# lorenzrichter/path-space-PDE-solver

Measured on AMD Instinct MI355X. Metric: trajectory-timesteps/sec (K*N/s), d=100 HJB log-variance training iteration, higher is better.
Workload: dtype f32 (f16x3 split products: every matrix product as three f16 MFMAs, fp32 accumulate; state / sums fp32)

## Files before the change

path-space-pde-solver_amd/csrc/hjb_kernels.h:

```cpp
#pragma once
#include <cstdlib>
#include <type_traits>
#include <hip/hip_runtime.h>
#include <stdint.h>

namespace psp {

typedef float f32x4 __attribute__((ext_vector_type(4)));

struct HjbArgs {
    const float* params;
    const float* x0;
    const float* y0;
    const float* xi;
    float* path;
    float* D;
    float* XN;
    double* fwd_partial;
    const float* drift;
    const float* sigma;
    const float* runcost;
    const float* term;
    const double* sums;
    float* grad_partial;
// ... 190 lines not shown
    constexpr int NCH = cdiv(KS, CH);
    lane = opaque_i(lane);
    float buf[2][CH * MB];
#pragma unroll
    for (int kk = 0; kk < CH; ++kk)
#pragma unroll
        for (int mb = 0; mb < MB; ++mb)
            if (kk < KS) buf[0][kk * MB + mb] = wlds[(mb * KS + kk) * 64 + lane];
#pragma unroll
    for (int c = 0; c < NCH; ++c) {
        if (c + 1 < NCH) {
#pragma unroll
            for (int kk = 0; kk < CH; ++kk)
#pragma unroll
                for (int mb = 0; mb < MB; ++mb) {
                    const int ks = (c + 1) * CH + kk;
                    if (ks < KS) buf[(c + 1) & 1][kk * MB + mb] = wlds[(mb * KS + ks) * 64 + lane];
                }
        }
#pragma unroll
        for (int kk = 0; kk < CH; ++kk) {
            const int ks = c * CH + kk;
            if (ks < KS) {
                const float bop = in[ks >> 2][ks & 3];
#pragma unroll
                for (int mb = 0; mb < MB; ++mb) acc[mb] = mfma16(buf[c & 1][kk * MB + mb], bop, acc[mb]);
            }
        }
        __builtin_amdgcn_sched_barrier(kFenceMask);
    }
}

typedef __bf16 bf16x8 __attribute__((ext_vector_type(8)));
template <class F>
__device__ __forceinline__ void stage_aop_bf16(float* dstf, int MB, int NS, int tid, int nthr, F src) {
    bf16x8* dst = reinterpret_cast<bf16x8*>(dstf);
    const int total = MB * NS * 64;
    for (int idx = tid; idx < total; idx += nthr) {
        const int lane = idx & 63, t = idx >> 6;
        const int S = t % NS, mb = t / NS;
        const int i = lane & 15, g = lane >> 4;
        const int row = 16 * mb + 4 * (i & 3) + (i >> 2);
        bf16x8 v;
#pragma unroll
        for (int e = 0; e < 8; ++e) v[e] = (__bf16)src(row, 32 * S + (e < 4 ? 4 * e : 16 + 4 * (e - 4)) + g);
        dst[idx] = v;
    }
}
template <int MB, int INB>
__device__ __forceinline__ void gemm_Tb(f32x4 (&acc)[MB], const float* wlds, const f32x4 (&in)[INB], int lane) {
    constexpr int NS = (INB + 1) / 2;
    const bf16x8* tbl = reinterpret_cast<const bf16x8*>(wlds) + opaque_i(lane);
#pragma unroll
    for (int S = 0; S < NS; ++S) {
        bf16x8 b;
#pragma unroll
        for (int e = 0; e < 4; ++e) {
            b[e] = (__bf16)in[2 * S][e];
            b[4 + e] = (2 * S + 1 < INB) ? (__bf16)in[(2 * S + 1 < INB) ? 2 * S + 1 : 0][e] : (__bf16)0.0f;
        }
#pragma unroll
        for (int mb = 0; mb < MB; ++mb)
            acc[mb] = __builtin_amdgcn_mfma_f32_16x16x32_bf16(tbl[(mb * NS + S) * 64], b, acc[mb], 0, 0, 0);
    }
}

typedef _Float16 f16x8 __attribute__((ext_vector_type(8)));
typedef _Float16 f16x4 __attribute__((ext_vector_type(4)));
constexpr float kSplitScale = 2048.0f, kSplitInv = 1.0f / 2048.0f;
template <int KS, int INB>
struct SplitGeo {
    static constexpr int NS = INB / 2;
    static constexpr bool ODD = (INB & 1) != 0;
    static constexpr int NKR = ODD ? KS - 8 * NS : 0;
    static constexpr bool ODD_F32 = ODD && NKR <= 1;
    static constexpr bool ODD_H16 = ODD && NKR > 1;
    static constexpr int per_mb = NS * 512 + (ODD_F32 ? 64 : 0) + (ODD_H16 ? 256 : 0);
    static constexpr int floats(int MB) { return MB * per_mb; }
};
__device__ __forceinline__ void split_f16(float v, _Float16& hi, _Float16& lo) {
    hi = (_Float16)v;
    lo = (_Float16)((v - (float)hi) * kSplitScale);
}

typedef _Float16 f16x2 __attribute__((ext_vector_type(2)));
typedef float f32x2 __attribute__((ext_vector_type(2)));
__device__ __forceinline__ void split_pair(float a, float b, f16x2& hi, f16x2& lo) {
    const f32x2 v = {a, b};
    hi = __builtin_convertvector(v, f16x2);
    const f32x2 s = v * kSplitScale;
    lo[0] = (_Float16)__builtin_fmaf((float)hi[0], -kSplitScale, s[0]);
    lo[1] = (_Float16)__builtin_fmaf((float)hi[1], -kSplitScale, s[1]);
}
__device__ __forceinline__ void split4c(const f32x4& u, f16x4& hi, f16x4& lo) {
#pragma unroll
    for (int e = 0; e < 4; ++e) {
        _Float16 h, l;
        split_f16(u[e], h, l);
        hi[e] = h; lo[e] = l;
    }
}
__device__ __forceinline__ void split4(const f32x4& u, f16x4& hi, f16x4& lo) {
#if defined(PSP_SPLIT_CLASSIC) && PSP_SPLIT_CLASSIC
#pragma unroll
    for (int e = 0; e < 4; ++e) {
        _Float16 h, l;
        split_f16(u[e], h, l);
        hi[e] = h; lo[e] = l;
    }
    return;
#endif
    f16x2 h, l;
    split_pair(u[0], u[1], h, l); hi[0] = h[0]; hi[1] = h[1]; lo[0] = l[0]; lo[1] = l[1];
    split_pair(u[2], u[3], h, l); hi[2] = h[0]; hi[3] = h[1]; lo[2] = l[0]; lo[3] = l[1];
}
__device__ __forceinline__ void split8(const f32x4& u0, const f32x4& u1, f16x8& hi, f16x8& lo) {
#if defined(PSP_SPLIT_CLASSIC) && PSP_SPLIT_CLASSIC
#pragma unroll
    for (int e = 0; e < 4; ++e) {
        _Float16 h, l;
        split_f16(u0[e], h, l);
        hi[e] = h; lo[e] = l;
        split_f16(u1[e], h, l);
        hi[4 + e] = h; lo[4 + e] = l;
    }
    return;
#endif
    f16x2 h, l;
    split_pair(u0[0], u0[1], h, l); hi[0] = h[0]; hi[1] = h[1]; lo[0] = l[0]; lo[1] = l[1];
    split_pair(u0[2], u0[3], h, l); hi[2] = h[0]; hi[3] = h[1]; lo[2] = l[0]; lo[3] = l[1];
    split_pair(u1[0], u1[1], h, l); hi[4] = h[0]; hi[5] = h[1]; lo[4] = l[0]; lo[5] = l[1];
    split_pair(u1[2], u1[3], h, l); hi[6] = h[0]; hi[7] = h[1]; lo[6] = l[0]; lo[7] = l[1];
}
__device__ __forceinline__ void split_pair_u(float a, float b, f16x2& hi, f16x2& lo) {
    const f32x2 v = {a, b};
    hi = __builtin_convertvector(v, f16x2);
    lo[0] = (_Float16)__builtin_fmaf((float)hi[0], -1.0f, v[0]);
    lo[1] = (_Float16)__builtin_fmaf((float)hi[1], -1.0f, v[1]);
}
__device__ __forceinline__ void split8u(const f32x4& u0, const f32x4& u1, f16x8& hi, f16x8& lo) {
#if defined(PSP_SPLIT_CLASSIC) && PSP_SPLIT_CLASSIC
#pragma unroll
    for (int e = 0; e < 4; ++e) {
        _Float16 h = (_Float16)u0[e];
        hi[e] = h; lo[e] = (_Float16)(u0[e] - (float)h);
        h = (_Float16)u1[e];
        hi[4 + e] = h; lo[4 + e] = (_Float16)(u1[e] - (float)h);
    }
    return;
#endif
    f16x2 h, l;
    split_pair_u(u0[0], u0[1], h, l); hi[0] = h[0]; hi[1] = h[1]; lo[0] = l[0]; lo[1] = l[1];
    split_pair_u(u0[2], u0[3], h, l); hi[2] = h[0]; hi[3] = h[1]; lo[2] = l[0]; lo[3] = l[1];
    split_pair_u(u1[0], u1[1], h, l); hi[4] = h[0]; hi[5] = h[1]; lo[4] = l[0]; lo[5] = l[1];
    split_pair_u(u1[2], u1[3], h, l); hi[6] = h[0]; hi[7] = h[1]; lo[6] = l[0]; lo[7] = l[1];
}
template <int KS, int INB, class F>
__device__ __forceinline__ void stage_aop_x3(float* dstf, int MB, int tid, int nthr, F src) {
    using SG = SplitGeo<KS, INB>;
    if constexpr (SG::NS > 0) {
        for (int idx = tid; idx < MB * SG::NS * 64; idx += nthr) {
            const int lane = idx & 63, t = idx >> 6;
            const int S = t % SG::NS, mb = t / SG::NS;
            const int i = lane & 15, g = lane >> 4;
            const int row = 16 * mb + 4 * (i & 3) + (i >> 2);
            f16x8 hi, lo;
#pragma unroll
            for (int e = 0; e < 8; ++e) {
                _Float16 h, l;
                split_f16(src(row, 32 * S + (e < 4 ? 4 * e : 16 + 4 * (e - 4)) + g), h, l);
                hi[e] = h; lo[e] = l;
            }
            f16x8* p = reinterpret_cast<f16x8*>(dstf + mb * SG::per_mb + S * 512);
            p[lane] = hi; p[64 + lane] = lo;
        }
    }
    if constexpr (SG::ODD) {
        for (int idx = tid; idx < MB * 64; idx += nthr) {
            const int lane = idx & 63, mb = idx >> 6;
            const int i = lane & 15, g = lane >> 4;
            const int row = 16 * mb + 4 * (i & 3) + (i >> 2);
            if constexpr (SG::ODD_F32) {
                dstf[mb * SG::per_mb + SG::NS * 512 + lane] = src(row, 32 * SG::NS + g);
            } else {
                f16x4 hi, lo;
#pragma unroll
                for (int e = 0; e < 4; ++e) {
                    _Float16 h, l;
                    split_f16(src(row, 32 * SG::NS + 4 * e + g), h, l);
                    hi[e] = h; lo[e] = l;
                }
                f16x4* p = reinterpret_cast<f16x4*>(dstf + mb * SG::per_mb + SG::NS * 512);
                p[lane] = hi; p[64 + lane] = lo;
            }
        }
    }
}
struct NoBetween { __device__ __forceinline__ void operator()(int) const {} };
template <int MB, int KS, int INB, int CU = 2, class BT = NoBetween>
__device__ __forceinline__ void gemm_Tx(f32x4 (&acc)[MB], const float* wlds, const f32x4 (&in)[INB], int lane, BT between = BT()) {
    constexpr int kFence = std::is_same<BT, NoBetween>::value ? kFenceMask : 0;
    using SG = SplitGeo<KS, INB>;
    constexpr int NS = SG::NS;
    static_assert(MB * SG::per_mb * 4 <= 65536, "table exceeds the 16-bit ds_read immediate offset");
    lane = opaque_i(lane);
    f32x4 corr[MB];
#pragma unroll
    for (int mb = 0; mb < MB; ++mb) corr[mb] = f32x4{0.f, 0.f, 0.f, 0.f};
    if constexpr (NS > 0) {
        const f16x8* tbl = reinterpret_cast<const f16x8*>(wlds) + lane;
        constexpr int NU = NS * MB, R = 2 * CU, PF = R - 1;
        f16x8 ah[R], al[R];
#pragma unroll
        for (int u = 0; u < PF; ++u)
            if (u < NU) {
                ah[u % R] = tbl[((u % MB) * SG::per_mb + (u / MB) * 512) / 4];
                al[u % R] = tbl[((u % MB) * SG::per_mb + (u / MB) * 512) / 4 + 64];
            }
        f16x8 bh, bl;
#pragma unroll
        for (int u = 0; u < NU; ++u) {
            if (u + PF < NU) {
                const int v = u + PF;
                ah[v % R] = tbl[((v % MB) * SG::per_mb + (v / MB) * 512) / 4];
                al[v % R] = tbl[((v % MB) * SG::per_mb + (v / MB) * 512) / 4 + 64];
            }
            const int S = u / MB, mb = u % MB;
            if (mb == 0) split8(in[2 * S], in[2 * S + 1], bh, bl);
            acc[mb] = __builtin_amdgcn_mfma_f32_16x16x32_f16(ah[u % R], bh, acc[mb], 0, 0, 0);
            corr[mb] = __builtin_amdgcn_mfma_f32_16x16x32_f16(ah[u % R], bl, corr[mb], 0, 0, 0);
            corr[mb] = __builtin_amdgcn_mfma_f32_16x16x32_f16(al[u % R], bh, corr[mb], 0, 0, 0);
            between(u);
            __builtin_amdgcn_sched_barrier(kFence);
        }
    }
    if constexpr (SG::ODD_F32) {
        const float bop = in[INB - 1][0];
#pragma unroll
        for (int mb = 0; mb < MB; ++mb) acc[mb] = mfma16(wlds[mb * SG::per_mb + NS * 512 + lane], bop, acc[mb]);
    }
    if constexpr (SG::ODD_H16) {
        f16x4 bh, bl;
        split4c(in[INB - 1], bh, bl);
#pragma unroll
        for (int mb = 0; mb < MB; ++mb) {
            const f16x4* p = reinterpret_cast<const f16x4*>(wlds + mb * SG::per_mb + NS * 512) + lane;
            const f16x4 a_hi = p[0], a_lo = p[64];
            acc[mb] = __builtin_amdgcn_mfma_f32_16x16x16f16(a_hi, bh, acc[mb], 0, 0, 0);
            corr[mb] = __builtin_amdgcn_mfma_f32_16x16x16f16(a_hi, bl, corr[mb], 0, 0, 0);
            corr[mb] = __builtin_amdgcn_mfma_f32_16x16x16f16(a_lo, bh, corr[mb], 0, 0, 0);
        }
    }
#pragma unroll
    for (int mb = 0; mb < MB; ++mb) acc[mb] = acc[mb] + kSplitInv * corr[mb];
}

template <int INB>
__device__ __forceinline__ void split_panel8(const f32x4 (&in)[INB], f16x8 (&bh)[INB / 2 > 0 ? INB / 2 : 1], f16x8 (&bl)[INB / 2 > 0 ? INB / 2 : 1]) {
#pragma unroll
    for (int S = 0; S < INB / 2; ++S) split8(in[2 * S], in[2 * S + 1], bh[S], bl[S]);
}
template <int MB, int KS, int INB, int CU = 2, class BT = NoBetween>
__device__ __forceinline__ void gemm_Txs(f32x4 (&acc)[MB], const float* wlds, const f16x8 (&bh)[INB / 2 > 0 ? INB / 2 : 1],
                                         const f16x8 (&bl)[INB / 2 > 0 ? INB / 2 : 1], const f32x4& last, int lane, BT between = BT()) {
    constexpr int kFence = std::is_same<BT, NoBetween>::value ? kFenceMask : 0;
    using SG = SplitGeo<KS, INB>;
    constexpr int NS = SG::NS;
    lane = opaque_i(lane);
    f32x4 corr[MB];
#pragma unroll
    for (int mb = 0; mb < MB; ++mb) corr[mb] = f32x4{0.f, 0.f, 0.f, 0.f};
    if constexpr (NS > 0) {
        const f16x8* tbl = reinterpret_cast<const f16x8*>(wlds) + lane;
        constexpr int NU = NS * MB, R = 2 * CU, PF = R - 1;
        f16x8 ah[R], al[R];
#pragma unroll
        for (int u = 0; u < PF; ++u)
            if (u < NU) {
                ah[u % R] = tbl[((u % MB) * SG::per_mb + (u / MB) * 512) / 4];
                al[u % R] = tbl[((u % MB) * SG::per_mb + (u / MB) * 512) / 4 + 64];
            }
#pragma unroll
        for (int u = 0; u < NU; ++u) {
            if (u + PF < NU) {
                const int v = u + PF;
                ah[v % R] = tbl[((v % MB) * SG::per_mb + (v / MB) * 512) / 4];
                al[v % R] = tbl[((v % MB) * SG::per_mb + (v / MB) * 512) / 4 + 64];
            }
            const int S = u / MB, mb = u % MB;
            acc[mb] = __builtin_amdgcn_mfma_f32_16x16x32_f16(ah[u % R], bh[S], acc[mb], 0, 0, 0);
            corr[mb] = __builtin_amdgcn_mfma_f32_16x16x32_f16(ah[u % R], bl[S], corr[mb], 0, 0, 0);
            corr[mb] = __builtin_amdgcn_mfma_f32_16x16x32_f16(al[u % R], bh[S], corr[mb], 0, 0, 0);
            between(u);
            __builtin_amdgcn_sched_barrier(kFence);
        }
    }
    if constexpr (SG::ODD_F32) {
        const float bop = last[0];
#pragma unroll
        for (int mb = 0; mb < MB; ++mb) acc[mb] = mfma16(wlds[mb * SG::per_mb + NS * 512 + lane], bop, acc[mb]);
    }
    if constexpr (SG::ODD_H16) {
        f16x4 b4h, b4l;
        split4c(last, b4h, b4l);
#pragma unroll
        for (int mb = 0; mb < MB; ++mb) {
            const f16x4* p = reinterpret_cast<const f16x4*>(wlds + mb * SG::per_mb + NS * 512) + lane;
            const f16x4 a_hi = p[0], a_lo = p[64];
            acc[mb] = __builtin_amdgcn_mfma_f32_16x16x16f16(a_hi, b4h, acc[mb], 0, 0, 0);
            corr[mb] = __builtin_amdgcn_mfma_f32_16x16x16f16(a_hi, b4l, corr[mb], 0, 0, 0);
            corr[mb] = __builtin_amdgcn_mfma_f32_16x16x16f16(a_lo, b4h, corr[mb], 0, 0, 0);
        }
    }
#pragma unroll
    for (int mb = 0; mb < MB; ++mb) acc[mb] = acc[mb] + kSplitInv * corr[mb];
}

__device__ __forceinline__ float qsum(float v) {
    v += __shfl_xor(v, 16);
    v += __shfl_xor(v, 32);
    return v;
}
__device__ __forceinline__ float jsumf(float v) {
    v += __shfl_xor(v, 1);
    v += __shfl_xor(v, 2);
    v += __shfl_xor(v, 4);
    v += __shfl_xor(v, 8);
    return v;
}
__device__ __forceinline__ double jsum(double v) {
    v += __shfl_xor(v, 1);
    v += __shfl_xor(v, 2);
    v += __shfl_xor(v, 4);
    v += __shfl_xor(v, 8);
    return v;
}

__device__ __forceinline__ float tanh_f32(float x) {
    const float e = __builtin_amdgcn_exp2f(fabsf(x) * 2.8853900817779268f);
    const float big = fmaf(-2.0f, __builtin_amdgcn_rcpf(e + 1.0f), 1.0f);
    return copysignf(big, x);
}
__device__ __forceinline__ f32x4 tanh4(f32x4 v) {
    f32x4 o;
    o[0] = tanh_f32(v[0]); o[1] = tanh_f32(v[1]); o[2] = tanh_f32(v[2]); o[3] = tanh_f32(v[3]);
    return o;
}

__device__ __forceinline__ f32x4 relu4n(f32x4 v) {
    f32x4 o;
    o[0] = v[0] < 0.f ? 0.f : v[0]; o[1] = v[1] < 0.f ? 0.f : v[1]; o[2] = v[2] < 0.f ? 0.f : v[2]; o[3] = v[3] < 0.f ? 0.f : v[3];
    return o;
}

template <int D, int H>
struct Geo {
    static constexpr int DB = cdiv(D, 16), HB = cdiv(H, 16);
    static constexpr int KSD = cdiv(D, 4), KSH = cdiv(H, 4);
    static constexpr int oW1 = 0, ob1 = H * (D + 1), oW2 = ob1 + H, ob2 = oW2 + H * H, oW3 = ob2 + H,
                         ob3 = oW3 + D * H, P = ob3 + D;
    static constexpr int tbl(int MB, int KS, int INB) { return MB * (KS > 4 * ((INB + 1) / 2) ? KS : 4 * ((INB + 1) / 2)) * 64; }
    static constexpr int fW1 = 0, fW2 = fW1 + tbl(HB, KSD, DB), fW3 = fW2 + tbl(HB, KSH, HB),
                         fVec = fW3 + tbl(DB, KSH, HB);
    static_assert(D <= 12 || H <= 12 || fVec == (HB * KSD + HB * KSH + DB * KSH) * 64, "only inputs of <= 12 features change the carve");
    static constexpr int vb1 = fVec, vw1t = vb1 + HB * 16, vb2 = vw1t + HB * 16, vb3 = vb2 + HB * 16,
                         vdr = vb3 + DB * 16, vrun = vdr + DB * 16, vterm = vrun + DB * 16,
                         fRed = vterm + DB * 16;
    static constexpr int fA = fRed + 64;
    static constexpr int fB_dense_off = DB * KSD * 64;
    static constexpr int xW1 = 0, xW2 = xW1 + SplitGeo<KSD, DB>::floats(HB), xW3 = xW2 + SplitGeo<KSH, HB>::floats(HB),
                         xVec = xW3 + SplitGeo<KSH, HB>::floats(DB), xA = xVec + (fA - fVec);
    static constexpr int xB_dense_off = SplitGeo<KSD, DB>::floats(DB);
    static int fwd_x3_lds_floats(int drift_kind, int sigma_kind) {
        return xA + (drift_kind == DRIFT_DENSE ? xB_dense_off : 0) + (sigma_kind == SIGMA_DENSE ? xB_dense_off : 0);
    }
    static int fwd_lds_floats(int drift_kind, int sigma_kind) {
        return fA + (drift_kind == DRIFT_DENSE ? fB_dense_off : 0) + (sigma_kind == SIGMA_DENSE ? fB_dense_off : 0);
    }
    static constexpr int pX = 0, pH1 = 4 * DB * 64, pH2 = pH1 + 4 * HB * 64, pXi = pH2 + 4 * HB * 64, PB = pXi + 4 * DB * 64;
    static constexpr int WH = (HB >= 4) ? 4 : (HB >= 2 ? 2 : 1);
    static constexpr int WD = 4 / WH;
    static constexpr int NIB = cdiv(HB, WH);
    static constexpr int NOBD = cdiv(DB, WD);
    static constexpr int NOBH = cdiv(HB, WD);
    static constexpr int EXB = KSD * 64 + 4 * HB * 64;
    static int bwd2_lds_floats() { return HB * KSD * 64 + 2 * 4 * EXB; }
};

template <int D, int H, int MODE = 0, int FAST_ = 0>
__global__ __launch_bounds__(512) void hjb_fwd_kernel(const HjbArgs a) {
    PSP_COND_EXIT(a);
    constexpr bool FAST = FAST_ != 0, SPEC = FAST_ >= 2;
    const int k_drift = SPEC ? (int)DRIFT_DENSE : a.drift_kind;
    const int k_sigma = FAST_ == 3 ? (int)SIGMA_IDENT : SPEC ? (int)SIGMA_DENSE : a.sigma_kind;
    const int k_run = SPEC ? (int)RUN_ZERO : a.runcost_kind, k_loss = SPEC ? (int)LOSS_LOGVAR : a.loss_kind;
    const int k_store = a.store_path;
    const bool k_adaptive = SPEC ? true : (a.adaptive != 0);
    const uint32_t iter_now = a.iter_dev ? *a.iter_dev : a.iter;
    using G = Geo<D, H>;
    constexpr int DB = G::DB, HB = G::HB, KSD = G::KSD, KSH = G::KSH;
    constexpr bool BF16 = MODE == 1, X3 = MODE == 2;
    constexpr int oW1 = X3 ? G::xW1 : G::fW1, oW2 = X3 ? G::xW2 : G::fW2, oW3 = X3 ? G::xW3 : G::fW3;
    constexpr int VEC = X3 ? G::xVec : G::fVec;
    constexpr int VSH = VEC - G::fVec;
    extern __shared__ __attribute__((aligned(16))) float lds[];
    const int tid = threadIdx.x, nthr = blockDim.x;
    const int lane = tid & 63, wave = tid >> 6, nwave = nthr >> 6;
    const int j = lane & 15, q = lane >> 4;

    const float* __restrict__ P = a.params;
    auto stage_net = [&](float* dst, int MB, int KS, int INB, auto src) {
        if constexpr (BF16) stage_aop_bf16(dst, MB, (INB + 1) / 2, tid, nthr, src);
        else stage_aop(dst, MB, KS, tid, nthr, src);
    };
    auto w1src = [&](int row, int col) { return (row < H && col < D) ? P[G::oW1 + row * (D + 1) + 1 + col] : 0.f; };
    auto w2src = [&](int row, int col) { return (row < H && col < H) ? P[G::oW2 + row * H + col] : 0.f; };
    auto w3src = [&](int row, int col) { return (row < D && col < H) ? P[G::oW3 + row * H + col] : 0.f; };
    if constexpr (X3) {
        stage_aop_x3<KSD, DB>(lds + oW1, HB, tid, nthr, w1src);
        stage_aop_x3<KSH, HB>(lds + oW2, HB, tid, nthr, w2src);
        stage_aop_x3<KSH, HB>(lds + oW3, DB, tid, nthr, w3src);
    } else {
        stage_net(lds + oW1, HB, KSD, DB, w1src);
        stage_net(lds + oW2, HB, KSH, HB, w2src);
        stage_net(lds + oW3, DB, KSH, HB, w3src);
    }
    float* ldsA = lds + G::fA + VSH;
    float* ldsB = ldsA + (k_drift == DRIFT_DENSE ? (X3 ? G::xB_dense_off : G::fB_dense_off) : 0);
    if (k_drift == DRIFT_DENSE) {
        const float dt = a.dt;
        const float* __restrict__ A = a.drift;
        auto asrc = [&](int row, int col) { return (row < D && col < D) ? dt * A[row * D + col] : 0.f; };
        if constexpr (X3) stage_aop_x3<KSD, DB>(ldsA, DB, tid, nthr, asrc);
        else stage_aop(ldsA, DB, KSD, tid, nthr, asrc);
    }
    if (k_sigma == SIGMA_DENSE) {
        const float* __restrict__ B = a.sigma;
        auto bsrc = [&](int row, int col) { return (row < D && col < D) ? B[row * D + col] : 0.f; };
        if constexpr (X3) stage_aop_x3<KSD, DB>(ldsB, DB, tid, nthr, bsrc);
        else stage_aop(ldsB, DB, KSD, tid, nthr, bsrc);
    }
    stage_vec(lds + VSH + G::vb1, HB, tid, nthr, [&](int f) { return f < H ? P[G::ob1 + f] : 0.f; });
    stage_vec(lds + VSH + G::vw1t, HB, tid, nthr, [&](int f) { return f < H ? P[G::oW1 + f * (D + 1)] : 0.f; });
    stage_vec(lds + VSH + G::vb2, HB, tid, nthr, [&](int f) { return f < H ? P[G::ob2 + f] : 0.f; });
    stage_vec(lds + VSH + G::vb3, DB, tid, nthr, [&](int f) { return f < D ? P[G::ob3 + f] : 0.f; });
    stage_vec(lds + VSH + G::vdr, DB, tid, nthr, [&](int f) {
        return (f < D && (k_drift == DRIFT_DIAG || k_drift == DRIFT_DWELL)) ? a.drift[f] : 0.f; });
    stage_vec(lds + VSH + G::vrun, DB, tid, nthr, [&](int f) {
        return (f < D && k_run == RUN_DIAGQ) ? a.runcost[f] : 0.f; });
    stage_vec(lds + VSH + G::vterm, DB, tid, nthr, [&](int f) { return f < D ? a.term[f] : 0.f; });
    __syncthreads();

    const int t16 = blockIdx.x * nwave + wave;
    const bool wave_valid = t16 < a.ntile16;
    const int k = t16 * 16 + j;
    const bool kvalid = wave_valid && k < a.K_local;
    const uint32_t kglob = (uint32_t)(a.k_offset + k);
    const float dt = a.dt, sqdt = a.sqdt;

    const float store_cxi = SPEC ? 1.f : ((k_store == 3) ? 0.f : 1.f);
    const float store_cz = SPEC ? 0.f : ((k_store == 3) ? 1.f : (k_store == 2 ? -a.sqdt : (k_adaptive ? 0.f : a.sqdt)));
    const bool do_store = FAST ? true : (k_store != 0);
    double sD = 0.0, sD2 = 0.0;
    if (wave_valid) {
        const f32x4* vecs0 = reinterpret_cast<const f32x4*>(lds + VEC) + q;
        const f32x4* vterm = vecs0 + (G::vterm - G::fVec) / 4;

        f32x4 X[DB];
#pragma unroll
        for (int b = 0; b < DB; ++b) {
#pragma unroll
            for (int r = 0; r < 4; ++r) {
                const int f = 16 * b + 4 * r + q;
                const float v = a.x0[(size_t)(kvalid ? k : 0) * a.x0_stride + (f < D ? f : D - 1)];
                X[b][r] = (f < D && kvalid) ? v : 0.f;
            }
        }
        float Y = a.y0 ? a.y0[0] : 0.f;
        float Fsum = 0.f, ULsum = 0.f;
#ifdef PSP_STAMPS
        unsigned long long stamps[8] = {0, 0, 0, 0, 0, 0, 0, 0};
#endif

        for (int n = 0; n < a.N; ++n) {
            PSP_STAMP(fs0);
            float tn = (float)n * dt;
            if constexpr (!FAST) { if (a.tfeat) tn = a.tfeat[n]; }
            const f32x4* vecs = opaque(vecs0);
            const f32x4* vb1 = vecs + (G::vb1 - G::fVec) / 4;
            const f32x4* vw1t = vecs + (G::vw1t - G::fVec) / 4;
            const f32x4* vb2 = vecs + (G::vb2 - G::fVec) / 4;
            const f32x4* vb3 = vecs + (G::vb3 - G::fVec) / 4;
            const f32x4* vdr = vecs + (G::vdr - G::fVec) / 4;
            const f32x4* vrun = vecs + (G::vrun - G::fVec) / 4;
            float* pblk = a.path + ((size_t)n * a.ntile16 + t16) * (size_t)G::PB + lane;
            auto x_store = [&](int u, int NU) __attribute__((always_inline)) {
                if (do_store) {
#pragma unroll
                    for (int ks = 0; ks < 4 * DB; ++ks)
                        if (ks >= u * (4 * DB) / NU && ks < (u + 1) * (4 * DB) / NU)
                            PSP_PATH_STORE(pblk + (G::pX / 64 + ks) * 64, X[ks >> 2][ks & 3]);
                }
            };
            if (!X3 && do_store) {
#pragma unroll
                for (int ks = 0; ks < 4 * DB; ++ks) PSP_PATH_STORE(pblk + (G::pX / 64 + ks) * 64, X[ks >> 2][ks & 3]);
            }
            f32x4 h1[HB];
#pragma unroll
            for (int m = 0; m < HB; ++m) h1[m] = vb1[m * 4] + tn * vw1t[m * 4];
            f32x4 Tn[DB];
            const bool early_drift = X3 && k_drift == DRIFT_DENSE;
            if constexpr (X3) {
                if (k_drift == DRIFT_DENSE) {
                    f16x8 xh[DB / 2 > 0 ? DB / 2 : 1], xl[DB / 2 > 0 ? DB / 2 : 1];
                    constexpr int NU1 = (DB / 2) * HB, NU2 = (DB / 2) * DB;
                    split_panel8<DB>(X, xh, xl);
                    gemm_Txs<HB, KSD, DB, 2>(h1, lds + oW1, xh, xl, X[DB - 1], lane, [&](int u) __attribute__((always_inline)) { x_store(u, NU1 + NU2); });
#pragma unroll
                    for (int b = 0; b < DB; ++b) Tn[b] = X[b];
                    gemm_Txs<DB, KSD, DB, 2>(Tn, ldsA, xh, xl, X[DB - 1], lane, [&](int u) __attribute__((always_inline)) { x_store(NU1 + u, NU1 + NU2); });
                    if constexpr (NU1 + NU2 == 0) x_store(0, 1);
                } else {
                    constexpr int NU1 = (DB / 2) * HB;
                    gemm_Tx<HB, KSD, DB, 2>(h1, lds + oW1, X, lane, [&](int u) __attribute__((always_inline)) { x_store(u, NU1); });
                    if constexpr (NU1 == 0) x_store(0, 1);
                }
            }
            else if constexpr (BF16) gemm_Tb<HB, DB>(h1, lds + oW1, X, lane);
            else gemm_T<HB, KSD, DB>(h1, lds + oW1, X, lane);
            PSP_STAMP(fs1);
#pragma unroll
            for (int m = 0; m < HB; ++m) h1[m] = tanh4(h1[m]);
            PSP_STAMP(fs2);
            f32x4 h2[HB];
#pragma unroll
            for (int m = 0; m < HB; ++m) h2[m] = vb2[m * 4];
            constexpr int NUH2 = (HB / 2) * HB, NUH3 = (HB / 2) * DB;
            constexpr bool PREGEN = X3 && FAST && (NUH2 + NUH3 > 0);
            [[maybe_unused]] f32x4 xig[PREGEN ? DB : 1];
            [[maybe_unused]] uint32_t pc0 = 0, pc1 = 0, pc2 = 0, pc3 = 0;
            constexpr int NSPC = kPhiloxRounds + 1;
            auto philox_slice = [&](int sidx) __attribute__((always_inline)) {
                const int b = sidx / NSPC, sub = sidx % NSPC;
                if (sub == 0) { pc0 = kglob; pc1 = (uint32_t)n; pc2 = (uint32_t)(4 * b + q); pc3 = iter_now; }
                if (sub < kPhiloxRounds) {
                    philox_round(pc0, pc1, pc2, pc3, a.seed_lo + (uint32_t)sub * 0x9E3779B9u, a.seed_hi + (uint32_t)sub * 0xBB67AE85u);
                    asm volatile("" : "+v"(pc0), "+v"(pc1), "+v"(pc2), "+v"(pc3));
                } else {
                    const uint32_t rr[4] = {pc0, pc1, pc2, pc3};
                    f32x4 xi = normal4(rr);
                    if (16 * b + 16 > D) {
#pragma unroll
                        for (int r = 0; r < 4; ++r) if (16 * b + 4 * r + q >= D) xi[r] = 0.f;
                    }
                    asm volatile("" : "+v"(xi));
                    xig[b < DB ? b : 0] = xi;
                }
            };
            auto philox_portion = [&](int u) __attribute__((always_inline)) {
                if constexpr (PREGEN) {
#pragma unroll
                    for (int sidx = 0; sidx < NSPC * DB; ++sidx)
                        if (sidx >= u * (NSPC * DB) / (NUH2 + NUH3) && sidx < (u + 1) * (NSPC * DB) / (NUH2 + NUH3)) philox_slice(sidx);
                }
            };
            auto h_store = [&](const f32x4 (&h)[HB], int slot, int u, int NU) __attribute__((always_inline)) {
                if (do_store) {
#pragma unroll
                    for (int ks = 0; ks < 4 * HB; ++ks)
                        if (ks >= u * (4 * HB) / NU && ks < (u + 1) * (4 * HB) / NU)
                            PSP_PATH_STORE(pblk + (slot / 64 + ks) * 64, h[ks >> 2][ks & 3]);
                }
            };
            if constexpr (X3) {
                gemm_Tx<HB, KSH, HB, 2>(h2, lds + oW2, h1, lane, [&](int u) __attribute__((always_inline)) { h_store(h1, G::pH1, u, NUH2); philox_portion(u); });
                if constexpr (NUH2 == 0) h_store(h1, G::pH1, 0, 1);
            }
            else if constexpr (BF16) gemm_Tb<HB, HB>(h2, lds + oW2, h1, lane);
            else gemm_T<HB, KSH, HB>(h2, lds + oW2, h1, lane);
#pragma unroll
            for (int m = 0; m < HB; ++m) h2[m] = tanh4(h2[m]);
            if (!X3 && do_store) {
#pragma unroll
                for (int ks = 0; ks < 4 * HB; ++ks) {
                    PSP_PATH_STORE(pblk + (G::pH1 / 64 + ks) * 64, h1[ks >> 2][ks & 3]);
                    PSP_PATH_STORE(pblk + (G::pH2 / 64 + ks) * 64, h2[ks >> 2][ks & 3]);
                }
            }
            f32x4 Z[DB];
#pragma unroll
            for (int m = 0; m < DB; ++m) Z[m] = vb3[m * 4];
            if constexpr (X3) {
                gemm_Tx<DB, KSH, HB, 2>(Z, lds + oW3, h2, lane, [&](int u) __attribute__((always_inline)) { h_store(h2, G::pH2, u, NUH3); philox_portion(NUH2 + u); });
                if constexpr (NUH3 == 0) h_store(h2, G::pH2, 0, 1);
            }
            else if constexpr (BF16) gemm_Tb<DB, HB>(Z, lds + oW3, h2, lane);
            else gemm_T<DB, KSH, HB>(Z, lds + oW3, h2, lane);
            PSP_STAMP(fs3);

            float S = 0.f, Pz = 0.f, UL = 0.f;
#pragma unroll
            for (int b = 0; b < DB; ++b) {
                f32x4 xi;
                if constexpr (PREGEN) {
                    xi = xig[b];
                } else if (FAST || a.noise_mode == NOISE_PHILOX) {
                    xi = philox_block(kglob, (uint32_t)n, (uint32_t)(4 * b + q), iter_now, a.seed_lo, a.seed_hi);
                } else {
                    const float* xrow = a.xi + ((size_t)(n + 1) * a.K_local + (kvalid ? k : 0)) * D;
#pragma unroll
                    for (int r = 0; r < 4; ++r) {
                        const int f = 16 * b + 4 * r + q;
                        const float v = xrow[f < D ? f : D - 1];
                        xi[r] = (f < D && kvalid) ? v : 0.f;
                    }
                }
                if (16 * b + 16 > D) {
#pragma unroll
                    for (int r = 0; r < 4; ++r) if (16 * b + 4 * r + q >= D) xi[r] = 0.f;
                }
                if (do_store && k_store != 4) {
                    const f32x4 wv = store_cxi * xi + store_cz * Z[b];
#pragma unroll
                    for (int r = 0; r < 4; ++r) PSP_PATH_STORE(pblk + (G::pXi / 64 + 4 * b + r) * 64, wv[r]);
                }
#pragma unroll
                for (int r = 0; r < 4; ++r) {
                    S = fmaf(Z[b][r], Z[b][r], S);
                    Pz = fmaf(Z[b][r], xi[r], Pz);
                }
                if (!FAST && a.uref) {
                    const float* ur = a.uref + (size_t)n * D;
#pragma unroll
                    for (int r = 0; r < 4; ++r) {
                        const int f = 16 * b + 4 * r + q;
                        const float e = (f < D) ? Z[b][r] + ur[f < D ? f : D - 1] : 0.f;
                        UL = fmaf(e, e, UL);
                    }
                }
                Z[b] = k_adaptive ? (sqdt * xi - dt * Z[b]) : (sqdt * xi);
            }
            ULsum = fmaf(UL, dt, ULsum);
            S = qsum(S);
            Pz = qsum(Pz);
            PSP_STAMP(fs4);

            if (!early_drift) {
#pragma unroll
                for (int b = 0; b < DB; ++b) Tn[b] = X[b];
            }
            if (k_drift == DRIFT_DENSE) {
                if constexpr (!X3) gemm_T<DB, KSD, DB>(Tn, ldsA, X, lane);
            } else if (k_drift == DRIFT_DIAG) {
#pragma unroll
                for (int b = 0; b < DB; ++b) Tn[b] += dt * (vdr[b * 4] * X[b]);
            } else if (k_drift == DRIFT_DWELL) {
#pragma unroll
                for (int b = 0; b < DB; ++b) Tn[b] -= dt * (4.0f * vdr[b * 4] * (X[b] * (X[b] * X[b] - 1.0f)));
            }
            if (k_sigma == SIGMA_DENSE) {
                if constexpr (X3) gemm_Tx<DB, KSD, DB>(Tn, ldsB, Z, lane);
                else gemm_T<DB, KSD, DB>(Tn, ldsB, Z, lane);
            } else if (k_sigma == SIGMA_SCALE) {
#pragma unroll
                for (int b = 0; b < DB; ++b) Tn[b] += a.sigma_scale * Z[b];
            } else {
#pragma unroll
                for (int b = 0; b < DB; ++b) Tn[b] += Z[b];
            }
#pragma unroll
            for (int b = 0; b < DB; ++b) X[b] = Tn[b];
            PSP_STAMP(fs5);

            float fX = 0.f;
            if (k_run == RUN_DIAGQ) {
#pragma unroll
                for (int b = 0; b < DB; ++b) {
                    const f32x4 pv = vrun[b * 4];
#pragma unroll
                    for (int r = 0; r < 4; ++r) fX = fmaf(pv[r] * X[b][r], X[b][r], fX);
                }
                fX = qsum(fX);
            }
            if (k_loss == LOSS_RELENT) {
                Y = Y - (0.5f * S + fX) * dt;
            } else {
                const float drift_y = k_adaptive ? (fX - 0.5f * S) : (fX + 0.5f * S);
                Y = Y + drift_y * dt + Pz * sqdt;
            }
            Fsum = fmaf(fX, dt, Fsum);
            PSP_STAMP(fs6);
            PSP_ACC(0, fs1, fs0);
            PSP_ACC(1, fs2, fs1);
            PSP_ACC(2, fs3, fs2);
            PSP_ACC(3, fs4, fs3);
            PSP_ACC(4, fs5, fs4);
            PSP_ACC(5, fs6, fs5);
            PSP_ACC(6, fs6, fs0);
        }
#ifdef PSP_STAMPS
        if (a.dbg && lane == 0) {
            stamps[7] = (unsigned long long)a.N;
            for (int i = 0; i < 8; ++i) a.dbg[((size_t)blockIdx.x * 8 + wave) * 8 + i] = stamps[i];
        }
#endif

        float g = 0.f;
#pragma unroll
        for (int b = 0; b < DB; ++b) {
            const f32x4 tv = vterm[b * 4];
#pragma unroll
            for (int r = 0; r < 4; ++r) {
                const float x = X[b][r];
                if (a.term_kind == TERM_LINEAR) g = fmaf(tv[r], x, g);
                else if (a.term_kind == TERM_DIAGQ) g = fmaf(tv[r] * x, x, g);
                else g = fmaf(tv[r] * (x - 1.0f), (x - 1.0f), g);
            }
        }
        g = qsum(g);
        const float Dk = Y - g;
        if (kvalid && q == 0) a.D[k] = Dk;
        if (a.Fint && kvalid && q == 0) a.Fint[k] = Fsum;
        if (a.uref) {
            const float ULt = qsum(ULsum);
            if (kvalid && q == 0) a.ul2[k] = ULt;
        }
        if (a.Yout && kvalid && q == 0) a.Yout[k] = Y;
        if (a.XN && kvalid) {
#pragma unroll
            for (int b = 0; b < DB; ++b)
#pragma unroll
                for (int r = 0; r < 4; ++r) {
                    const int f = 16 * b + 4 * r + q;
                    if (f < D) a.XN[(size_t)k * D + f] = X[b][r];
                }
        }
        if (kvalid && q == 0) { sD = (double)Dk; sD2 = (double)Dk * (double)Dk; }
    }
    sD = jsum(sD); sD2 = jsum(sD2);
    double* red = reinterpret_cast<double*>(lds + G::fRed + VSH);
    if (lane == 0) { red[2 * wave] = sD; red[2 * wave + 1] = sD2; }
    __syncthreads();
    if (tid == 0) {
        double t0 = 0.0, t1 = 0.0;
// ... 452 lines not shown
```

Measured before the change: 1.862 billion.

## Pre-scale split operands so all three f16 MFMA terms share one accumulator

The weight tables are pre-scaled by 2^6 and the activation operands by 2^5 at split time, so the hi*lo and lo*hi correction products come out at the same 2048x scale as the main product. All three MFMAs can then accumulate into a single register set, which removes the separate corr accumulators and the final rescale-and-add. The 2048 scale is then undone downstream: biases are staged pre-scaled, tanh folds 1/2048 into its exponent, and the Z, S, Pz, drift and sigma paths get explicit 1/2048 factors. This cuts accumulator register pressure and per-GEMM VALU work, at the cost of a changed rounding profile and many scale-bookkeeping sites that must all stay consistent.

```diff
diff --git a/path-space-pde-solver_amd/csrc/hjb_kernels.h b/path-space-pde-solver_amd/csrc/hjb_kernels.h
--- a/path-space-pde-solver_amd/csrc/hjb_kernels.h
+++ b/path-space-pde-solver_amd/csrc/hjb_kernels.h
@@ -296,6 +296,19 @@
     hi = (_Float16)v;
     lo = (_Float16)((v - (float)hi) * kSplitScale);
 }
+constexpr int kLgFwdA = 6, kLgFwdB = 5;
+static_assert(kLgFwdA + kLgFwdB == 11, "p + q = 11: the accumulators hold 2048 a b");
+__host__ __device__ constexpr float pow2f(int e) { return e >= 0 ? (float)(1 << e) : 1.0f / (float)(1 << -e); }
+template <int LG>
+__device__ __forceinline__ void split_tab(float v, _Float16& hi, _Float16& lo) {
+    if constexpr (LG >= 0) {
+        const float s = pow2f(LG) * v;
+        hi = (_Float16)s;
+        lo = (_Float16)(s - (float)hi);
+    } else {
+        split_f16(v, hi, lo);
+    }
+}
 
 typedef _Float16 f16x2 __attribute__((ext_vector_type(2)));
 typedef float f32x2 __attribute__((ext_vector_type(2)));
@@ -369,7 +382,35 @@
     split_pair_u(u1[0], u1[1], h, l); hi[4] = h[0]; hi[5] = h[1]; lo[4] = l[0]; lo[5] = l[1];
     split_pair_u(u1[2], u1[3], h, l); hi[6] = h[0]; hi[7] = h[1]; lo[6] = l[0]; lo[7] = l[1];
 }
-template <int KS, int INB, class F>
+__device__ __forceinline__ void split_pair_s(float a, float b, float c, f16x2& hi, f16x2& lo) {
+    const f32x2 s = f32x2{a, b} * c;
+    hi = __builtin_convertvector(s, f16x2);
+    float m1 = -1.0f;
+    asm("" : "+s"(m1));
+    lo[0] = (_Float16)__builtin_fmaf((float)hi[0], m1, s[0]);
+    lo[1] = (_Float16)__builtin_fmaf((float)hi[1], m1, s[1]);
+}
+__device__ __forceinline__ void split4s(const f32x4& u, float c, f16x4& hi, f16x4& lo) {
+    f16x2 h, l;
+    split_pair_s(u[0], u[1], c, h, l); hi[0] = h[0]; hi[1] = h[1]; lo[0] = l[0]; lo[1] = l[1];
+    split_pair_s(u[2], u[3], c, h, l); hi[2] = h[0]; hi[3] = h[1]; lo[2] = l[0]; lo[3] = l[1];
+}
+__device__ __forceinline__ void split8s(const f32x4& u0, const f32x4& u1, float c, f16x8& hi, f16x8& lo) {
+    f16x4 h0, l0, h1, l1;
+    split4s(u0, c, h0, l0);
+    split4s(u1, c, h1, l1);
+    hi = __builtin_shufflevector(h0, h1, 0, 1, 2, 3, 4, 5, 6, 7);
+    lo = __builtin_shufflevector(l0, l1, 0, 1, 2, 3, 4, 5, 6, 7);
+}
+__device__ __forceinline__ void split4cs(const f32x4& u, float c, f16x4& hi, f16x4& lo) {
+#pragma unroll
+    for (int e = 0; e < 4; ++e) {
+        const float s = c * u[e];
+        const _Float16 h = (_Float16)s;
+        hi[e] = h; lo[e] = (_Float16)(s - (float)h);
+    }
+}
+template <int KS, int INB, int LG = -1, class F>
 __device__ __forceinline__ void stage_aop_x3(float* dstf, int MB, int tid, int nthr, F src) {
     using SG = SplitGeo<KS, INB>;
     if constexpr (SG::NS > 0) {
@@ -382,7 +423,7 @@
 #pragma unroll
             for (int e = 0; e < 8; ++e) {
                 _Float16 h, l;
-                split_f16(src(row, 32 * S + (e < 4 ? 4 * e : 16 + 4 * (e - 4)) + g), h, l);
+                split_tab<LG>(src(row, 32 * S + (e < 4 ? 4 * e : 16 + 4 * (e - 4)) + g), h, l);
                 hi[e] = h; lo[e] = l;
             }
             f16x8* p = reinterpret_cast<f16x8*>(dstf + mb * SG::per_mb + S * 512);
@@ -395,13 +436,13 @@
             const int i = lane & 15, g = lane >> 4;
             const int row = 16 * mb + 4 * (i & 3) + (i >> 2);
             if constexpr (SG::ODD_F32) {
-                dstf[mb * SG::per_mb + SG::NS * 512 + lane] = src(row, 32 * SG::NS + g);
+                dstf[mb * SG::per_mb + SG::NS * 512 + lane] = (LG >= 0 ? pow2f(LG) : 1.0f) * src(row, 32 * SG::NS + g);
             } else {
                 f16x4 hi, lo;
 #pragma unroll
                 for (int e = 0; e < 4; ++e) {
                     _Float16 h, l;
-                    split_f16(src(row, 32 * SG::NS + 4 * e + g), h, l);
+                    split_tab<LG>(src(row, 32 * SG::NS + 4 * e + g), h, l);
                     hi[e] = h; lo[e] = l;
                 }
                 f16x4* p = reinterpret_cast<f16x4*>(dstf + mb * SG::per_mb + SG::NS * 512);
@@ -411,16 +452,18 @@
     }
 }
 struct NoBetween { __device__ __forceinline__ void operator()(int) const {} };
-template <int MB, int KS, int INB, int CU = 2, class BT = NoBetween>
+template <int MB, int KS, int INB, int CU = 2, bool ONE = false, class BT = NoBetween>
 __device__ __forceinline__ void gemm_Tx(f32x4 (&acc)[MB], const float* wlds, const f32x4 (&in)[INB], int lane, BT between = BT()) {
     constexpr int kFence = std::is_same<BT, NoBetween>::value ? kFenceMask : 0;
     using SG = SplitGeo<KS, INB>;
     constexpr int NS = SG::NS;
     static_assert(MB * SG::per_mb * 4 <= 65536, "table exceeds the 16-bit ds_read immediate offset");
     lane = opaque_i(lane);
-    f32x4 corr[MB];
-#pragma unroll
-    for (int mb = 0; mb < MB; ++mb) corr[mb] = f32x4{0.f, 0.f, 0.f, 0.f};
+    [[maybe_unused]] f32x4 corr[ONE ? 1 : MB];
+    if constexpr (!ONE) {
+#pragma unroll
+        for (int mb = 0; mb < MB; ++mb) corr[mb] = f32x4{0.f, 0.f, 0.f, 0.f};
+    }
     if constexpr (NS > 0) {
         const f16x8* tbl = reinterpret_cast<const f16x8*>(wlds) + lane;
         constexpr int NU = NS * MB, R = 2 * CU, PF = R - 1;
@@ -440,39 +483,55 @@
                 al[v % R] = tbl[((v % MB) * SG::per_mb + (v / MB) * 512) / 4 + 64];
             }
             const int S = u / MB, mb = u % MB;
-            if (mb == 0) split8(in[2 * S], in[2 * S + 1], bh, bl);
+            if (mb == 0) {
+                if constexpr (ONE) split8s(in[2 * S], in[2 * S + 1], pow2f(kLgFwdB), bh, bl);
+                else split8(in[2 * S], in[2 * S + 1], bh, bl);
+            }
             acc[mb] = __builtin_amdgcn_mfma_f32_16x16x32_f16(ah[u % R], bh, acc[mb], 0, 0, 0);
-            corr[mb] = __builtin_amdgcn_mfma_f32_16x16x32_f16(ah[u % R], bl, corr[mb], 0, 0, 0);
-            corr[mb] = __builtin_amdgcn_mfma_f32_16x16x32_f16(al[u % R], bh, corr[mb], 0, 0, 0);
+            if constexpr (ONE) {
+                acc[mb] = __builtin_amdgcn_mfma_f32_16x16x32_f16(ah[u % R], bl, acc[mb], 0, 0, 0);
+                acc[mb] = __builtin_amdgcn_mfma_f32_16x16x32_f16(al[u % R], bh, acc[mb], 0, 0, 0);
+            } else {
+                corr[mb] = __builtin_amdgcn_mfma_f32_16x16x32_f16(ah[u % R], bl, corr[mb], 0, 0, 0);
+                corr[mb] = __builtin_amdgcn_mfma_f32_16x16x32_f16(al[u % R], bh, corr[mb], 0, 0, 0);
+            }
             between(u);
             __builtin_amdgcn_sched_barrier(kFence);
         }
     }
     if constexpr (SG::ODD_F32) {
-        const float bop = in[INB - 1][0];
+        const float bop = (ONE ? pow2f(kLgFwdB) : 1.0f) * in[INB - 1][0];
 #pragma unroll
         for (int mb = 0; mb < MB; ++mb) acc[mb] = mfma16(wlds[mb * SG::per_mb + NS * 512 + lane], bop, acc[mb]);
     }
     if constexpr (SG::ODD_H16) {
         f16x4 bh, bl;
-        split4c(in[INB - 1], bh, bl);
+        if constexpr (ONE) split4cs(in[INB - 1], pow2f(kLgFwdB), bh, bl);
+        else split4c(in[INB - 1], bh, bl);
 #pragma unroll
         for (int mb = 0; mb < MB; ++mb) {
             const f16x4* p = reinterpret_cast<const f16x4*>(wlds + mb * SG::per_mb + NS * 512) + lane;
             const f16x4 a_hi = p[0], a_lo = p[64];
             acc[mb] = __builtin_amdgcn_mfma_f32_16x16x16f16(a_hi, bh, acc[mb], 0, 0, 0);
-            corr[mb] = __builtin_amdgcn_mfma_f32_16x16x16f16(a_hi, bl, corr[mb], 0, 0, 0);
-            corr[mb] = __builtin_amdgcn_mfma_f32_16x16x16f16(a_lo, bh, corr[mb], 0, 0, 0);
-        }
-    }
-#pragma unroll
-    for (int mb = 0; mb < MB; ++mb) acc[mb] = acc[mb] + kSplitInv * corr[mb];
+            if constexpr (ONE) {
+                acc[mb] = __builtin_amdgcn_mfma_f32_16x16x16f16(a_hi, bl, acc[mb], 0, 0, 0);
+                acc[mb] = __builtin_amdgcn_mfma_f32_16x16x16f16(a_lo, bh, acc[mb], 0, 0, 0);
+            } else {
+                corr[mb] = __builtin_amdgcn_mfma_f32_16x16x16f16(a_hi, bl, corr[mb], 0, 0, 0);
+                corr[mb] = __builtin_amdgcn_mfma_f32_16x16x16f16(a_lo, bh, corr[mb], 0, 0, 0);
+            }
+        }
+    }
+    if constexpr (!ONE) {
+#pragma unroll
+        for (int mb = 0; mb < MB; ++mb) acc[mb] = acc[mb] + kSplitInv * corr[mb];
+    }
 }
 
 template <int INB>
 __device__ __forceinline__ void split_panel8(const f32x4 (&in)[INB], f16x8 (&bh)[INB / 2 > 0 ? INB / 2 : 1], f16x8 (&bl)[INB / 2 > 0 ? INB / 2 : 1]) {
 #pragma unroll
-    for (int S = 0; S < INB / 2; ++S) split8(in[2 * S], in[2 * S + 1], bh[S], bl[S]);
+    for (int S = 0; S < INB / 2; ++S) split8s(in[2 * S], in[2 * S + 1], pow2f(kLgFwdB), bh[S], bl[S]);
 }
 template <int MB, int KS, int INB, int CU = 2, class BT = NoBetween>
 __device__ __forceinline__ void gemm_Txs(f32x4 (&acc)[MB], const float* wlds, const f16x8 (&bh)[INB / 2 > 0 ? INB / 2 : 1],
@@ -481,9 +540,6 @@
     using SG = SplitGeo<KS, INB>;
     constexpr int NS = SG::NS;
     lane = opaque_i(lane);
-    f32x4 corr[MB];
-#pragma unroll
-    for (int mb = 0; mb < MB; ++mb) corr[mb] = f32x4{0.f, 0.f, 0.f, 0.f};
     if constexpr (NS > 0) {
         const f16x8* tbl = reinterpret_cast<const f16x8*>(wlds) + lane;
         constexpr int NU = NS * MB, R = 2 * CU, PF = R - 1;
@@ -503,31 +559,29 @@
             }
             const int S = u / MB, mb = u % MB;
             acc[mb] = __builtin_amdgcn_mfma_f32_16x16x32_f16(ah[u % R], bh[S], acc[mb], 0, 0, 0);
-            corr[mb] = __builtin_amdgcn_mfma_f32_16x16x32_f16(ah[u % R], bl[S], corr[mb], 0, 0, 0);
-            corr[mb] = __builtin_amdgcn_mfma_f32_16x16x32_f16(al[u % R], bh[S], corr[mb], 0, 0, 0);
+            acc[mb] = __builtin_amdgcn_mfma_f32_16x16x32_f16(ah[u % R], bl[S], acc[mb], 0, 0, 0);
+            acc[mb] = __builtin_amdgcn_mfma_f32_16x16x32_f16(al[u % R], bh[S], acc[mb], 0, 0, 0);
             between(u);
             __builtin_amdgcn_sched_barrier(kFence);
         }
     }
     if constexpr (SG::ODD_F32) {
-        const float bop = last[0];
+        const float bop = pow2f(kLgFwdB) * last[0];
 #pragma unroll
         for (int mb = 0; mb < MB; ++mb) acc[mb] = mfma16(wlds[mb * SG::per_mb + NS * 512 + lane], bop, acc[mb]);
     }
     if constexpr (SG::ODD_H16) {
         f16x4 b4h, b4l;
-        split4c(last, b4h, b4l);
+        split4cs(last, pow2f(kLgFwdB), b4h, b4l);
 #pragma unroll
         for (int mb = 0; mb < MB; ++mb) {
             const f16x4* p = reinterpret_cast<const f16x4*>(wlds + mb * SG::per_mb + NS * 512) + lane;
             const f16x4 a_hi = p[0], a_lo = p[64];
             acc[mb] = __builtin_amdgcn_mfma_f32_16x16x16f16(a_hi, b4h, acc[mb], 0, 0, 0);
-            corr[mb] = __builtin_amdgcn_mfma_f32_16x16x16f16(a_hi, b4l, corr[mb], 0, 0, 0);
-            corr[mb] = __builtin_amdgcn_mfma_f32_16x16x16f16(a_lo, b4h, corr[mb], 0, 0, 0);
-        }
-    }
-#pragma unroll
-    for (int mb = 0; mb < MB; ++mb) acc[mb] = acc[mb] + kSplitInv * corr[mb];
+            acc[mb] = __builtin_amdgcn_mfma_f32_16x16x16f16(a_hi, b4l, acc[mb], 0, 0, 0);
+            acc[mb] = __builtin_amdgcn_mfma_f32_16x16x16f16(a_lo, b4h, acc[mb], 0, 0, 0);
+        }
+    }
 }
 
 __device__ __forceinline__ float qsum(float v) {
@@ -550,14 +604,16 @@
     return v;
 }
 
+template <bool X2048 = false>
 __device__ __forceinline__ float tanh_f32(float x) {
-    const float e = __builtin_amdgcn_exp2f(fabsf(x) * 2.8853900817779268f);
+    const float e = __builtin_amdgcn_exp2f(fabsf(x) * (X2048 ? 2.8853900817779268f * kSplitInv : 2.8853900817779268f));
     const float big = fmaf(-2.0f, __builtin_amdgcn_rcpf(e + 1.0f), 1.0f);
     return copysignf(big, x);
 }
+template <bool X2048 = false>
 __device__ __forceinline__ f32x4 tanh4(f32x4 v) {
     f32x4 o;
-    o[0] = tanh_f32(v[0]); o[1] = tanh_f32(v[1]); o[2] = tanh_f32(v[2]); o[3] = tanh_f32(v[3]);
+    o[0] = tanh_f32<X2048>(v[0]); o[1] = tanh_f32<X2048>(v[1]); o[2] = tanh_f32<X2048>(v[2]); o[3] = tanh_f32<X2048>(v[3]);
     return o;
 }
 
@@ -631,9 +687,9 @@
     auto w2src = [&](int row, int col) { return (row < H && col < H) ? P[G::oW2 + row * H + col] : 0.f; };
     auto w3src = [&](int row, int col) { return (row < D && col < H) ? P[G::oW3 + row * H + col] : 0.f; };
     if constexpr (X3) {
-        stage_aop_x3<KSD, DB>(lds + oW1, HB, tid, nthr, w1src);
-        stage_aop_x3<KSH, HB>(lds + oW2, HB, tid, nthr, w2src);
-        stage_aop_x3<KSH, HB>(lds + oW3, DB, tid, nthr, w3src);
+        stage_aop_x3<KSD, DB, kLgFwdA>(lds + oW1, HB, tid, nthr, w1src);
+        stage_aop_x3<KSH, HB, kLgFwdA>(lds + oW2, HB, tid, nthr, w2src);
+        stage_aop_x3<KSH, HB, kLgFwdA>(lds + oW3, DB, tid, nthr, w3src);
     } else {
         stage_net(lds + oW1, HB, KSD, DB, w1src);
         stage_net(lds + oW2, HB, KSH, HB, w2src);
@@ -645,19 +701,20 @@
         const float dt = a.dt;
         const float* __restrict__ A = a.drift;
         auto asrc = [&](int row, int col) { return (row < D && col < D) ? dt * A[row * D + col] : 0.f; };
-        if constexpr (X3) stage_aop_x3<KSD, DB>(ldsA, DB, tid, nthr, asrc);
+        if constexpr (X3) stage_aop_x3<KSD, DB, kLgFwdA>(ldsA, DB, tid, nthr, asrc);
         else stage_aop(ldsA, DB, KSD, tid, nthr, asrc);
     }
     if (k_sigma == SIGMA_DENSE) {
         const float* __restrict__ B = a.sigma;
         auto bsrc = [&](int row, int col) { return (row < D && col < D) ? B[row * D + col] : 0.f; };
-        if constexpr (X3) stage_aop_x3<KSD, DB>(ldsB, DB, tid, nthr, bsrc);
+        if constexpr (X3) stage_aop_x3<KSD, DB, kLgFwdA>(ldsB, DB, tid, nthr, bsrc);
         else stage_aop(ldsB, DB, KSD, tid, nthr, bsrc);
     }
-    stage_vec(lds + VSH + G::vb1, HB, tid, nthr, [&](int f) { return f < H ? P[G::ob1 + f] : 0.f; });
-    stage_vec(lds + VSH + G::vw1t, HB, tid, nthr, [&](int f) { return f < H ? P[G::oW1 + f * (D + 1)] : 0.f; });
-    stage_vec(lds + VSH + G::vb2, HB, tid, nthr, [&](int f) { return f < H ? P[G::ob2 + f] : 0.f; });
-    stage_vec(lds + VSH + G::vb3, DB, tid, nthr, [&](int f) { return f < D ? P[G::ob3 + f] : 0.f; });
+    constexpr float kAcc = X3 ? kSplitScale : 1.0f, kAccInv = X3 ? kSplitInv : 1.0f;
+    stage_vec(lds + VSH + G::vb1, HB, tid, nthr, [&](int f) { return f < H ? kAcc * P[G::ob1 + f] : 0.f; });
+    stage_vec(lds + VSH + G::vw1t, HB, tid, nthr, [&](int f) { return f < H ? kAcc * P[G::oW1 + f * (D + 1)] : 0.f; });
+    stage_vec(lds + VSH + G::vb2, HB, tid, nthr, [&](int f) { return f < H ? kAcc * P[G::ob2 + f] : 0.f; });
+    stage_vec(lds + VSH + G::vb3, DB, tid, nthr, [&](int f) { return f < D ? kAcc * P[G::ob3 + f] : 0.f; });
     stage_vec(lds + VSH + G::vdr, DB, tid, nthr, [&](int f) {
         return (f < D && (k_drift == DRIFT_DIAG || k_drift == DRIFT_DWELL)) ? a.drift[f] : 0.f; });
     stage_vec(lds + VSH + G::vrun, DB, tid, nthr, [&](int f) {
@@ -673,7 +730,7 @@
     const float dt = a.dt, sqdt = a.sqdt;
 
     const float store_cxi = SPEC ? 1.f : ((k_store == 3) ? 0.f : 1.f);
-    const float store_cz = SPEC ? 0.f : ((k_store == 3) ? 1.f : (k_store == 2 ? -a.sqdt : (k_adaptive ? 0.f : a.sqdt)));
+    const float store_cz = kAccInv * (SPEC ? 0.f : ((k_store == 3) ? 1.f : (k_store == 2 ? -a.sqdt : (k_adaptive ? 0.f : a.sqdt))));
     const bool do_store = FAST ? true : (k_store != 0);
     double sD = 0.0, sD2 = 0.0;
     if (wave_valid) {
@@ -732,12 +789,12 @@
                     split_panel8<DB>(X, xh, xl);
                     gemm_Txs<HB, KSD, DB, 2>(h1, lds + oW1, xh, xl, X[DB - 1], lane, [&](int u) __attribute__((always_inline)) { x_store(u, NU1 + NU2); });
 #pragma unroll
-                    for (int b = 0; b < DB; ++b) Tn[b] = X[b];
+                    for (int b = 0; b < DB; ++b) Tn[b] = f32x4{0.f, 0.f, 0.f, 0.f};
                     gemm_Txs<DB, KSD, DB, 2>(Tn, ldsA, xh, xl, X[DB - 1], lane, [&](int u) __attribute__((always_inline)) { x_store(NU1 + u, NU1 + NU2); });
                     if constexpr (NU1 + NU2 == 0) x_store(0, 1);
                 } else {
                     constexpr int NU1 = (DB / 2) * HB;
-                    gemm_Tx<HB, KSD, DB, 2>(h1, lds + oW1, X, lane, [&](int u) __attribute__((always_inline)) { x_store(u, NU1); });
+                    gemm_Tx<HB, KSD, DB, 2, true>(h1, lds + oW1, X, lane, [&](int u) __attribute__((always_inline)) { x_store(u, NU1); });
                     if constexpr (NU1 == 0) x_store(0, 1);
                 }
             }
@@ -745,7 +802,7 @@
             else gemm_T<HB, KSD, DB>(h1, lds + oW1, X, lane);
             PSP_STAMP(fs1);
 #pragma unroll
-            for (int m = 0; m < HB; ++m) h1[m] = tanh4(h1[m]);
+            for (int m = 0; m < HB; ++m) h1[m] = tanh4<X3>(h1[m]);
             PSP_STAMP(fs2);
             f32x4 h2[HB];
 #pragma unroll
@@ -788,13 +845,13 @@
                 }
             };
             if constexpr (X3) {
-                gemm_Tx<HB, KSH, HB, 2>(h2, lds + oW2, h1, lane, [&](int u) __attribute__((always_inline)) { h_store(h1, G::pH1, u, NUH2); philox_portion(u); });
+                gemm_Tx<HB, KSH, HB, 2, true>(h2, lds + oW2, h1, lane, [&](int u) __attribute__((always_inline)) { h_store(h1, G::pH1, u, NUH2); philox_portion(u); });
                 if constexpr (NUH2 == 0) h_store(h1, G::pH1, 0, 1);
             }
             else if constexpr (BF16) gemm_Tb<HB, HB>(h2, lds + oW2, h1, lane);
             else gemm_T<HB, KSH, HB>(h2, lds + oW2, h1, lane);
 #pragma unroll
-            for (int m = 0; m < HB; ++m) h2[m] = tanh4(h2[m]);
+            for (int m = 0; m < HB; ++m) h2[m] = tanh4<X3>(h2[m]);
             if (!X3 && do_store) {
 #pragma unroll
                 for (int ks = 0; ks < 4 * HB; ++ks) {
@@ -806,7 +863,7 @@
 #pragma unroll
             for (int m = 0; m < DB; ++m) Z[m] = vb3[m * 4];
             if constexpr (X3) {
-                gemm_Tx<DB, KSH, HB, 2>(Z, lds + oW3, h2, lane, [&](int u) __attribute__((always_inline)) { h_store(h2, G::pH2, u, NUH3); philox_portion(NUH2 + u); });
+                gemm_Tx<DB, KSH, HB, 2, true>(Z, lds + oW3, h2, lane, [&](int u) __attribute__((always_inline)) { h_store(h2, G::pH2, u, NUH3); philox_portion(NUH2 + u); });
                 if constexpr (NUH3 == 0) h_store(h2, G::pH2, 0, 1);
             }
             else if constexpr (BF16) gemm_Tb<DB, HB>(Z, lds + oW3, h2, lane);
@@ -849,20 +906,25 @@
 #pragma unroll
                     for (int r = 0; r < 4; ++r) {
                         const int f = 16 * b + 4 * r + q;
-                        const float e = (f < D) ? Z[b][r] + ur[f < D ? f : D - 1] : 0.f;
+                        const float e = (f < D) ? (X3 ? fmaf(Z[b][r], kSplitInv, ur[f < D ? f : D - 1]) : Z[b][r] + ur[f < D ? f : D - 1]) : 0.f;
                         UL = fmaf(e, e, UL);
                     }
                 }
-                Z[b] = k_adaptive ? (sqdt * xi - dt * Z[b]) : (sqdt * xi);
+                if constexpr (X3) Z[b] = k_adaptive ? (sqdt * xi - (dt * kSplitInv) * Z[b]) : (sqdt * xi);
+                else Z[b] = k_adaptive ? (sqdt * xi - dt * Z[b]) : (sqdt * xi);
             }
             ULsum = fmaf(UL, dt, ULsum);
             S = qsum(S);
             Pz = qsum(Pz);
+            if constexpr (X3) { S *= kSplitInv * kSplitInv; Pz *= kSplitInv; }
             PSP_STAMP(fs4);
 
             if (!early_drift) {
 #pragma unroll
                 for (int b = 0; b < DB; ++b) Tn[b] = X[b];
+            } else {
+#pragma unroll
+                for (int b = 0; b < DB; ++b) Tn[b] = X[b] + kSplitInv * Tn[b];
             }
             if (k_drift == DRIFT_DENSE) {
                 if constexpr (!X3) gemm_T<DB, KSD, DB>(Tn, ldsA, X, lane);
@@ -874,7 +936,14 @@
                 for (int b = 0; b < DB; ++b) Tn[b] -= dt * (4.0f * vdr[b * 4] * (X[b] * (X[b] * X[b] - 1.0f)));
             }
             if (k_sigma == SIGMA_DENSE) {
-                if constexpr (X3) gemm_Tx<DB, KSD, DB>(Tn, ldsB, Z, lane);
+                if constexpr (X3) {
+                    f32x4 Bv[DB];
+#pragma unroll
+                    for (int b = 0; b < DB; ++b) Bv[b] = f32x4{0.f, 0.f, 0.f, 0.f};
+                    gemm_Tx<DB, KSD, DB, 2, true>(Bv, ldsB, Z, lane);
+#pragma unroll
+                    for (int b = 0; b < DB; ++b) Tn[b] = Tn[b] + kSplitInv * Bv[b];
+                }
                 else gemm_T<DB, KSD, DB>(Tn, ldsB, Z, lane);
             } else if (k_sigma == SIGMA_SCALE) {
 #pragma unroll
```

After: 1.884 billion, median of 6. +1.2%, better.
